# nexus-rl/dfd-starter

Measured on AMD Instinct MI355X. Metric: env steps/sec (whole node) + sec/FD-grad-step, 4096 antithetic perturbations, higher is better.
Workload: dtype f32; 1 GPU; BASELINE config 3: HalfCheetah-shaped synthetic env (obs 17, act 6), MujocoPolicy(17,6) P=6092, 4096 antithetic perturbations per GPU (2048 directions x +/-), T=1000 fixed-length episodes, full FD step (rollout + weights + gradient + DSGD); perturbations_per_gpu=4096, envs_per_perturbation=1, global_perturbations=4096, episode_len=1000, n_params=6092, parallelism=dp1

## Files before the change

### dfd-starter_amd/csrc/fdr_dpp_gen.h

```cpp
#pragma once

namespace fdr {

__device__ __forceinline__ void dpp_dot_32x1(float& a0, float X0, float X1, const float* w) {
  asm volatile(
      "s_nop 1\n\t"
      "v_mul_f32_dpp %0, %1, %3 row_newbcast:0 row_mask:0xf bank_mask:0xf\n\t"
      "v_fmac_f32_dpp %0, %2, %19 row_newbcast:0 row_mask:0xf bank_mask:0xf\n\t"
      "v_fmac_f32_dpp %0, %1, %4 row_newbcast:1 row_mask:0xf bank_mask:0xf\n\t"
      "v_fmac_f32_dpp %0, %2, %20 row_newbcast:1 row_mask:0xf bank_mask:0xf\n\t"
      "v_fmac_f32_dpp %0, %1, %5 row_newbcast:2 row_mask:0xf bank_mask:0xf\n\t"
      "v_fmac_f32_dpp %0, %2, %21 row_newbcast:2 row_mask:0xf bank_mask:0xf\n\t"
      "v_fmac_f32_dpp %0, %1, %6 row_newbcast:3 row_mask:0xf bank_mask:0xf\n\t"
      "v_fmac_f32_dpp %0, %2, %22 row_newbcast:3 row_mask:0xf bank_mask:0xf\n\t"
      "v_fmac_f32_dpp %0, %1, %7 row_newbcast:4 row_mask:0xf bank_mask:0xf\n\t"
      "v_fmac_f32_dpp %0, %2, %23 row_newbcast:4 row_mask:0xf bank_mask:0xf\n\t"
      "v_fmac_f32_dpp %0, %1, %8 row_newbcast:5 row_mask:0xf bank_mask:0xf\n\t"
      "v_fmac_f32_dpp %0, %2, %24 row_newbcast:5 row_mask:0xf bank_mask:0xf\n\t"
      "v_fmac_f32_dpp %0, %1, %9 row_newbcast:6 row_mask:0xf bank_mask:0xf\n\t"
      "v_fmac_f32_dpp %0, %2, %25 row_newbcast:6 row_mask:0xf bank_mask:0xf\n\t"
      "v_fmac_f32_dpp %0, %1, %10 row_newbcast:7 row_mask:0xf bank_mask:0xf\n\t"
      "v_fmac_f32_dpp %0, %2, %26 row_newbcast:7 row_mask:0xf bank_mask:0xf\n\t"
      "v_fmac_f32_dpp %0, %1, %11 row_newbcast:8 row_mask:0xf bank_mask:0xf\n\t"
      "v_fmac_f32_dpp %0, %2, %27 row_newbcast:8 row_mask:0xf bank_mask:0xf\n\t"
// ... 166 lines not shown
      "v_fmac_f32_dpp %0, %1, %11 row_newbcast:9 row_mask:0xf bank_mask:0xf\n\t"
      "v_fmac_f32_dpp %0, %1, %12 row_newbcast:10 row_mask:0xf bank_mask:0xf\n\t"
      : "+v"(a0)
      : "v"(X0), "v"(w[0]), "v"(w[1]), "v"(w[2]), "v"(w[3]), "v"(w[4]), "v"(w[5]), "v"(w[6]), "v"(w[7]), "v"(w[8]), "v"(w[9]), "v"(w[10]));
}
__device__ __forceinline__ void dpp_fma_tail12(float& a0, float X0, const float* w) {
  asm volatile(
      "s_nop 1\n\t"
      "v_fmac_f32_dpp %0, %1, %2 row_newbcast:0 row_mask:0xf bank_mask:0xf\n\t"
      "v_fmac_f32_dpp %0, %1, %3 row_newbcast:1 row_mask:0xf bank_mask:0xf\n\t"
      "v_fmac_f32_dpp %0, %1, %4 row_newbcast:2 row_mask:0xf bank_mask:0xf\n\t"
      "v_fmac_f32_dpp %0, %1, %5 row_newbcast:3 row_mask:0xf bank_mask:0xf\n\t"
      "v_fmac_f32_dpp %0, %1, %6 row_newbcast:4 row_mask:0xf bank_mask:0xf\n\t"
      "v_fmac_f32_dpp %0, %1, %7 row_newbcast:5 row_mask:0xf bank_mask:0xf\n\t"
      "v_fmac_f32_dpp %0, %1, %8 row_newbcast:6 row_mask:0xf bank_mask:0xf\n\t"
      "v_fmac_f32_dpp %0, %1, %9 row_newbcast:7 row_mask:0xf bank_mask:0xf\n\t"
      "v_fmac_f32_dpp %0, %1, %10 row_newbcast:8 row_mask:0xf bank_mask:0xf\n\t"
      "v_fmac_f32_dpp %0, %1, %11 row_newbcast:9 row_mask:0xf bank_mask:0xf\n\t"
      "v_fmac_f32_dpp %0, %1, %12 row_newbcast:10 row_mask:0xf bank_mask:0xf\n\t"
      "v_fmac_f32_dpp %0, %1, %13 row_newbcast:11 row_mask:0xf bank_mask:0xf\n\t"
      : "+v"(a0)
      : "v"(X0), "v"(w[0]), "v"(w[1]), "v"(w[2]), "v"(w[3]), "v"(w[4]), "v"(w[5]), "v"(w[6]), "v"(w[7]), "v"(w[8]), "v"(w[9]), "v"(w[10]), "v"(w[11]));
}
__device__ __forceinline__ void dpp_fma_tail13(float& a0, float X0, const float* w) {
  asm volatile(
      "s_nop 1\n\t"
      "v_fmac_f32_dpp %0, %1, %2 row_newbcast:0 row_mask:0xf bank_mask:0xf\n\t"
      "v_fmac_f32_dpp %0, %1, %3 row_newbcast:1 row_mask:0xf bank_mask:0xf\n\t"
      "v_fmac_f32_dpp %0, %1, %4 row_newbcast:2 row_mask:0xf bank_mask:0xf\n\t"
      "v_fmac_f32_dpp %0, %1, %5 row_newbcast:3 row_mask:0xf bank_mask:0xf\n\t"
      "v_fmac_f32_dpp %0, %1, %6 row_newbcast:4 row_mask:0xf bank_mask:0xf\n\t"
      "v_fmac_f32_dpp %0, %1, %7 row_newbcast:5 row_mask:0xf bank_mask:0xf\n\t"
      "v_fmac_f32_dpp %0, %1, %8 row_newbcast:6 row_mask:0xf bank_mask:0xf\n\t"
      "v_fmac_f32_dpp %0, %1, %9 row_newbcast:7 row_mask:0xf bank_mask:0xf\n\t"
      "v_fmac_f32_dpp %0, %1, %10 row_newbcast:8 row_mask:0xf bank_mask:0xf\n\t"
      "v_fmac_f32_dpp %0, %1, %11 row_newbcast:9 row_mask:0xf bank_mask:0xf\n\t"
      "v_fmac_f32_dpp %0, %1, %12 row_newbcast:10 row_mask:0xf bank_mask:0xf\n\t"
      "v_fmac_f32_dpp %0, %1, %13 row_newbcast:11 row_mask:0xf bank_mask:0xf\n\t"
      "v_fmac_f32_dpp %0, %1, %14 row_newbcast:12 row_mask:0xf bank_mask:0xf\n\t"
      : "+v"(a0)
      : "v"(X0), "v"(w[0]), "v"(w[1]), "v"(w[2]), "v"(w[3]), "v"(w[4]), "v"(w[5]), "v"(w[6]), "v"(w[7]), "v"(w[8]), "v"(w[9]), "v"(w[10]), "v"(w[11]), "v"(w[12]));
}
__device__ __forceinline__ void dpp_fma_tail14(float& a0, float X0, const float* w) {
  asm volatile(
      "s_nop 1\n\t"
      "v_fmac_f32_dpp %0, %1, %2 row_newbcast:0 row_mask:0xf bank_mask:0xf\n\t"
      "v_fmac_f32_dpp %0, %1, %3 row_newbcast:1 row_mask:0xf bank_mask:0xf\n\t"
      "v_fmac_f32_dpp %0, %1, %4 row_newbcast:2 row_mask:0xf bank_mask:0xf\n\t"
      "v_fmac_f32_dpp %0, %1, %5 row_newbcast:3 row_mask:0xf bank_mask:0xf\n\t"
      "v_fmac_f32_dpp %0, %1, %6 row_newbcast:4 row_mask:0xf bank_mask:0xf\n\t"
      "v_fmac_f32_dpp %0, %1, %7 row_newbcast:5 row_mask:0xf bank_mask:0xf\n\t"
      "v_fmac_f32_dpp %0, %1, %8 row_newbcast:6 row_mask:0xf bank_mask:0xf\n\t"
      "v_fmac_f32_dpp %0, %1, %9 row_newbcast:7 row_mask:0xf bank_mask:0xf\n\t"
      "v_fmac_f32_dpp %0, %1, %10 row_newbcast:8 row_mask:0xf bank_mask:0xf\n\t"
      "v_fmac_f32_dpp %0, %1, %11 row_newbcast:9 row_mask:0xf bank_mask:0xf\n\t"
      "v_fmac_f32_dpp %0, %1, %12 row_newbcast:10 row_mask:0xf bank_mask:0xf\n\t"
      "v_fmac_f32_dpp %0, %1, %13 row_newbcast:11 row_mask:0xf bank_mask:0xf\n\t"
      "v_fmac_f32_dpp %0, %1, %14 row_newbcast:12 row_mask:0xf bank_mask:0xf\n\t"
      "v_fmac_f32_dpp %0, %1, %15 row_newbcast:13 row_mask:0xf bank_mask:0xf\n\t"
      : "+v"(a0)
      : "v"(X0), "v"(w[0]), "v"(w[1]), "v"(w[2]), "v"(w[3]), "v"(w[4]), "v"(w[5]), "v"(w[6]), "v"(w[7]), "v"(w[8]), "v"(w[9]), "v"(w[10]), "v"(w[11]), "v"(w[12]), "v"(w[13]));
}
__device__ __forceinline__ void dpp_fma_tail15(float& a0, float X0, const float* w) {
  asm volatile(
      "s_nop 1\n\t"
      "v_fmac_f32_dpp %0, %1, %2 row_newbcast:0 row_mask:0xf bank_mask:0xf\n\t"
      "v_fmac_f32_dpp %0, %1, %3 row_newbcast:1 row_mask:0xf bank_mask:0xf\n\t"
      "v_fmac_f32_dpp %0, %1, %4 row_newbcast:2 row_mask:0xf bank_mask:0xf\n\t"
      "v_fmac_f32_dpp %0, %1, %5 row_newbcast:3 row_mask:0xf bank_mask:0xf\n\t"
      "v_fmac_f32_dpp %0, %1, %6 row_newbcast:4 row_mask:0xf bank_mask:0xf\n\t"
      "v_fmac_f32_dpp %0, %1, %7 row_newbcast:5 row_mask:0xf bank_mask:0xf\n\t"
      "v_fmac_f32_dpp %0, %1, %8 row_newbcast:6 row_mask:0xf bank_mask:0xf\n\t"
      "v_fmac_f32_dpp %0, %1, %9 row_newbcast:7 row_mask:0xf bank_mask:0xf\n\t"
      "v_fmac_f32_dpp %0, %1, %10 row_newbcast:8 row_mask:0xf bank_mask:0xf\n\t"
      "v_fmac_f32_dpp %0, %1, %11 row_newbcast:9 row_mask:0xf bank_mask:0xf\n\t"
      "v_fmac_f32_dpp %0, %1, %12 row_newbcast:10 row_mask:0xf bank_mask:0xf\n\t"
      "v_fmac_f32_dpp %0, %1, %13 row_newbcast:11 row_mask:0xf bank_mask:0xf\n\t"
      "v_fmac_f32_dpp %0, %1, %14 row_newbcast:12 row_mask:0xf bank_mask:0xf\n\t"
      "v_fmac_f32_dpp %0, %1, %15 row_newbcast:13 row_mask:0xf bank_mask:0xf\n\t"
      "v_fmac_f32_dpp %0, %1, %16 row_newbcast:14 row_mask:0xf bank_mask:0xf\n\t"
      : "+v"(a0)
      : "v"(X0), "v"(w[0]), "v"(w[1]), "v"(w[2]), "v"(w[3]), "v"(w[4]), "v"(w[5]), "v"(w[6]), "v"(w[7]), "v"(w[8]), "v"(w[9]), "v"(w[10]), "v"(w[11]), "v"(w[12]), "v"(w[13]), "v"(w[14]));
}
}
```

### dfd-starter_amd/csrc/fdr_mlp_pair.h

```cpp
#pragma once
#include "fdr_mlp.h"

namespace fdr {

constexpr int kPairWaves = 2;

__device__ __forceinline__ f2 tanh2_pre(f2 t) {
  const f2 d = f2{__builtin_amdgcn_exp2f(t.x), __builtin_amdgcn_exp2f(t.y)} + f2{1.f, 1.f};
  return pk_fma(f2{-2.f, -2.f}, f2{__builtin_amdgcn_rcpf(d.x), __builtin_amdgcn_rcpf(d.y)}, f2{1.f, 1.f});
}
__device__ __forceinline__ f2 tanh2_fast(f2 x) {
  return tanh2_pre(x * f2{kTanhScale, kTanhScale});
}
constexpr float kPreScale = kTanhScale;
template <bool kPre>
__device__ __forceinline__ f2 tanh2_act(f2 z) {
  if constexpr (kPre) return tanh2_pre(z);
  else return tanh2_fast(z);
}

template <int NIN, int NA, bool DISC>
struct MlpPair {
  using L = Layout<NIN, NA, DISC>;
  static constexpr int NOUT = L::NOUT;
  static constexpr int NX = round4(NIN);
  static_assert(NX <= 32, "pair kernel: policy input wider than 32");
  static constexpr bool kBiasCol = NIN < NX;
  static constexpr bool kW1Lds = NIN > 8;
  static constexpr bool kPre = !DISC;
  static constexpr float kWS = kPre ? kTanhScale : 1.f;
  static constexpr int kW1Chunks = kW1Lds ? NX / 4 : 0;
  static constexpr int kTileF4 = (2 * kW1Chunks + 8) * kWave;
  f2 w1a[kW1Lds ? 1 : NX / 2], w1b[kW1Lds ? 1 : NX / 2];
  float b1a, b1b;
  const float4* tile;
  f2 w2[64];
  float b2a, b2b, b3;
  float a0, c0, a1a, c1a, a1b, c1b, a2a, c2a, a2b, c2b;

  __host__ __device__ static constexpr int head_unit(int rho, int k, int e) {
    return 32 * rho + 8 * (k >> 2) + 4 * e + (k & 3);
  }

  template <class Src>
  __device__ __forceinline__ void load(Src& src, int t, int tid, const float* bn_mean, const float* bn_var,
                                       float4* wave_tile) {
    const int rho = t >> 4, o = t & 15;
    const int ua = 2 * t, ub = 2 * t + 1;
    float4* my = wave_tile + tid;
    tile = my;
    auto w1v = [&](int u, int k) {
      return kWS * (k < NIN ? src.get(L::L1W + (int64_t)u * NIN + k) : (k == NIN ? src.get(L::L1B + u) : 0.f));
    };
    if constexpr (kPk) {
#pragma unroll
      for (int j = 0; j < 2 * kW1Chunks; ++j) {
        const float e0 = w1v(ua, 2 * j), f0 = w1v(ub, 2 * j), e1 = w1v(ua, 2 * j + 1), f1 = w1v(ub, 2 * j + 1);
        my[j * kWave] = float4{e0, f0, e1, f1};
      }
    } else if constexpr (kW1Lds) {
#pragma unroll
      for (int m = 0; m < kW1Chunks; ++m) {
        const float e0 = w1v(ua, 4 * m), e1 = w1v(ua, 4 * m + 1), e2 = w1v(ua, 4 * m + 2), e3 = w1v(ua, 4 * m + 3);
        my[m * kWave] = float4{e0, e1, e2, e3};
        const float f0 = w1v(ub, 4 * m), f1 = w1v(ub, 4 * m + 1), f2_ = w1v(ub, 4 * m + 2), f3 = w1v(ub, 4 * m + 3);
        my[(kW1Chunks + m) * kWave] = float4{f0, f1, f2_, f3};
      }
    } else {
#pragma unroll
      for (int p = 0; p < NX / 2; ++p) {
        const float e0 = w1v(ua, 2 * p), e1 = w1v(ua, 2 * p + 1);
        w1a[p] = f2{e0, e1};
        const float f0 = w1v(ub, 2 * p), f1 = w1v(ub, 2 * p + 1);
        w1b[p] = f2{f0, f1};
      }
    }
    b1a = kBiasCol ? 0.f : kWS * src.get(L::L1B + ua);
    b1b = kBiasCol ? 0.f : kWS * src.get(L::L1B + ub);
    __builtin_amdgcn_sched_barrier(0);
    const int q4 = t >> 2, c4 = t & 3;
#pragma unroll
    for (int p = 0; p < 4; ++p) {
      const int row0 = 8 * q4 + (c4 ^ p), row1 = row0 + 4;
#pragma unroll
      for (int k = 0; k < 16; ++k) {
        const float e0 = src.get(L::L2W + (int64_t)row0 * kHidden + 16 * c4 + k);
        const float e1 = src.get(L::L2W + (int64_t)row1 * kHidden + 16 * c4 + k);
        w2[p * 16 + k] = f2{kWS * e0, kWS * e1};
      }
#pragma unroll
      for (int k = 0; k < 16; ++k) asm volatile("" : "+v"(w2[p * 16 + k]));
      asm volatile("" : "+v"(src.n2));
      __builtin_amdgcn_sched_barrier(0);
    }
    const int u2a = 8 * q4 + c4, u2b = 8 * q4 + 4 + c4;
    b2a = kWS * src.get(L::L2B + u2a);
    b2b = kWS * src.get(L::L2B + u2b);
    {
      const bool has_o = o < NOUT;
      const int oc = has_o ? o : 0;
#pragma unroll
      for (int m = 0; m < 8; ++m) {
        float e[4];
#pragma unroll
        for (int i = 0; i < 4; ++i) {
          const int w = 4 * m + i;
          e[i] = src.get_if(L::L3W + (int64_t)oc * kHidden + head_unit(rho, w & 15, w >> 4), has_o);
        }
        my[(2 * kW1Chunks + m) * kWave] =
            has_o ? float4{kWS * e[0], kWS * e[1], kWS * e[2], kWS * e[3]} : float4{0.f, 0.f, 0.f, 0.f};
      }
      const float b3v = src.get_if(L::L3B + oc, has_o && rho == 0);
      b3 = has_o ? kWS * b3v : 0.f;
    }
    wave_lds_sync();
    a0 = c0 = a1a = c1a = a1b = c1b = a2a = c2a = a2b = c2b = 0.f;
    if constexpr (DISC) {
      const float* bm = bn_mean ? bn_mean : src.base;
      const float* bv = bn_var ? bn_var : src.base;
      auto stat = [&](int k, float& rm, float& rv) {
        const float m = bm[k], v = bv[k];
        rm = bn_mean ? m : 0.f;
        rv = bn_var ? v : 1.f;
      };
      {
        const bool in = t < NIN;
        const int tc = in ? t : 0;
        const float w = src.get_if(L::BN0W + tc, in), b = src.get_if(L::BN0B + tc, in);
        float rm, rv, a, c;
        stat(tc, rm, rv);
        bn_fold(w, b, rm, rv, a, c);
        a0 = in ? a : 0.f;
        c0 = in ? c : 0.f;
      }
      auto fold = [&](int64_t wofs, int64_t bofs, int st, int u, float& av, float& cv) {
        const float w = src.get(wofs + u), b = src.get(bofs + u);
        float rm, rv;
        stat(st + u, rm, rv);
        bn_fold(w, b, rm, rv, av, cv);
      };
      fold(L::BN1W, L::BN1B, NIN, ua, a1a, c1a);
      fold(L::BN1W, L::BN1B, NIN, ub, a1b, c1b);
      fold(L::BN2W, L::BN2B, NIN + kHidden, u2a, a2a, c2a);
      fold(L::BN2W, L::BN2B, NIN + kHidden, u2b, a2b, c2b);
    }
  }

  __device__ __forceinline__ float input_transform(float x) const {
    if constexpr (DISC) {
      return fmaf(x, a0, c0);
    } else {
      return x;
    }
  }

  __device__ __forceinline__ float act1(float z, float av, float cv) const {
    if constexpr (DISC) {
      return fmaf(fmaxf(z, 0.f), av, cv);
    } else {
      return tanh_act<kPre>(z);
    }
  }

  static constexpr bool kTail = kW1Lds && kBiasCol && NX - NIN == 3;
  static constexpr int NQ = kTail ? NX / 4 - 1 : NX / 4;
  static constexpr bool kPk = kW1Lds && kBiasCol;
  static constexpr int kPkPairs = (NIN + 2) / 2;
  struct L1Rows {
    float4 wa[kW1Lds && !kPk ? NQ : 1], wb[kW1Lds && !kPk ? NQ : 1], m[NQ];
    float2 ta, tb;
    float tm;
    float4 wp[kPk ? kPkPairs : 1];
  };
  __device__ __forceinline__ void l1_prefetch(L1Rows& r, const float* mrow) const {
    const float4* m4 = reinterpret_cast<const float4*>(mrow);
#pragma unroll
    for (int q = 0; q < NQ; ++q) {
      if constexpr (kW1Lds && !kPk) {
        r.wa[q] = tile[q * kWave];
        r.wb[q] = tile[(kW1Chunks + q) * kWave];
      }
// ... 43 lines not shown
    const f2 am = am0 + am1;
    return am.x + am.y;
  }
  __device__ __forceinline__ f2 layer1_q(const SIn& xin, const L1Rows& rows) const {
    const float xt = xin.t;
    auto xq = [&](int q) { return xin.v[q]; };
    f2 aa0 = {b1a, 0.f}, aa1 = {0.f, 0.f}, ab0 = {b1b, 0.f}, ab1 = {0.f, 0.f};
    if constexpr (kPk) {
      constexpr int NC = 2;
      f2 acc[NC];
#pragma unroll
      for (int q = 0; q < NC; ++q) acc[q] = f2{0.f, 0.f};
#pragma unroll
      for (int q = 0; q < NQ; ++q) {
        const float4 xv = xq(q);
#pragma unroll
        for (int i = 0; i < 4; ++i) {
          const int k = 4 * q + i;
          if (k < NIN) {
            const float4 w = rows.wp[k >> 1];
            const f2 xp = (i < 2) ? f2{xv.x, xv.y} : f2{xv.z, xv.w};
            if (kPre && k == NIN % NC) {
              const float4 wb = rows.wp[NIN >> 1];
              const f2 bias = (NIN & 1) ? f2{wb.z, wb.w} : f2{wb.x, wb.y};
              acc[k % NC] = (k & 1) ? pk_fma_bhi(f2{w.z, w.w}, xp, bias) : pk_fma_blo(f2{w.x, w.y}, xp, bias);
            } else if (k < NC)
              acc[k % NC] = (k & 1) ? pk_mul_bhi(f2{w.z, w.w}, xp) : pk_mul_blo(f2{w.x, w.y}, xp);
            else
              acc[k % NC] = (k & 1) ? pk_fma_bhi(f2{w.z, w.w}, xp, acc[k % NC]) : pk_fma_blo(f2{w.x, w.y}, xp, acc[k % NC]);
          }
        }
      }
      if constexpr (kTail) {
        const float4 w = rows.wp[(NIN - 1) >> 1];
        acc[(NIN - 1) % NC] = pk_fma(((NIN - 1) & 1) ? f2{w.z, w.w} : f2{w.x, w.y}, f2{xt, xt}, acc[(NIN - 1) % NC]);
      }
      if constexpr (!kPre || NIN % NC >= NIN) {
        const float4 w = rows.wp[NIN >> 1];
        acc[NIN % NC] = acc[NIN % NC] + ((NIN & 1) ? f2{w.z, w.w} : f2{w.x, w.y});
      }
      const f2 h = acc[0] + acc[1];
      if constexpr (DISC) {
        return f2{act1(h.x, a1a, c1a), act1(h.y, a1b, c1b)};
      } else {
        return tanh2_act<kPre>(h);
      }
    }
#pragma unroll
    for (int q = 0; q < NQ; ++q) {
      const float4 xv = xq(q);
      float4 wa, wb;
      if constexpr (kW1Lds) {
        wa = rows.wa[q];
        wb = rows.wb[q];
      } else {
        wa = float4{w1a[2 * q].x, w1a[2 * q].y, w1a[2 * q + 1].x, w1a[2 * q + 1].y};
        wb = float4{w1b[2 * q].x, w1b[2 * q].y, w1b[2 * q + 1].x, w1b[2 * q + 1].y};
      }
      aa0 = pk_fma(f2{wa.x, wa.y}, f2{xv.x, xv.y}, aa0);
      ab0 = pk_fma(f2{wb.x, wb.y}, f2{xv.x, xv.y}, ab0);
      aa1 = pk_fma(f2{wa.z, wa.w}, f2{xv.z, xv.w}, aa1);
      ab1 = pk_fma(f2{wb.z, wb.w}, f2{xv.z, xv.w}, ab1);
    }
    if constexpr (kTail) {
      aa1 = pk_fma(f2{rows.ta.x, rows.ta.y}, f2{xt, 1.f}, aa1);
      ab1 = pk_fma(f2{rows.tb.x, rows.tb.y}, f2{xt, 1.f}, ab1);
    }
    const f2 ha = aa0 + aa1, hb = ab0 + ab1;
    if constexpr (DISC) {
      return f2{act1(ha.x + ha.y, a1a, c1a), act1(hb.x + hb.y, a1b, c1b)};
    } else {
      return tanh2_act<kPre>(f2{ha.x + ha.y, hb.x + hb.y});
    }
  }

  template <class Mark>
  __device__ __forceinline__ float layers23(f2 h1, float* h1s, int t, Mark&& mark) const {
    const int c4 = t & 3;
    float x[16];
    reinterpret_cast<f2*>(h1s)[t] = h1;
    __builtin_amdgcn_s_setprio(0);
    wave_lds_sync();
    lds_bcast<16>(h1s + 16 * c4, x);
    float w3[32];
#pragma unroll
    for (int m = 0; m < 8; ++m) {
      const float4 w = tile[(2 * kW1Chunks + m) * kWave];
      w3[4 * m] = w.x;
      w3[4 * m + 1] = w.y;
      w3[4 * m + 2] = w.z;
      w3[4 * m + 3] = w.w;
    }
    f2 acc[4];
#pragma unroll
    for (int p = 0; p < 4; ++p)
      acc[p] = pk_fma(w2[p * 16], f2{x[0], x[0]}, (kPre && p == 0) ? f2{b2a, b2b} : f2{0.f, 0.f});
    {
      f2 xp[8];
#pragma unroll
      for (int j = 0; j < 8; ++j) xp[j] = f2{x[2 * j], x[2 * j + 1]};
#define FDR_L2_HI "op_sel:[0,1,0] op_sel_hi:[1,1,1]"
#define FDR_L2_LO "op_sel_hi:[1,0,1]"
      asm(
          "v_pk_fma_f32 %0, %4, %64, %0 " FDR_L2_HI "\n"
          "v_pk_fma_f32 %1, %5, %64, %1 " FDR_L2_HI "\n"
          "v_pk_fma_f32 %2, %6, %64, %2 " FDR_L2_HI "\n"
          "v_pk_fma_f32 %3, %7, %64, %3 " FDR_L2_HI "\n"
          "v_pk_fma_f32 %0, %8, %65, %0 " FDR_L2_LO "\n"
          "v_pk_fma_f32 %1, %9, %65, %1 " FDR_L2_LO "\n"
          "v_pk_fma_f32 %2, %10, %65, %2 " FDR_L2_LO "\n"
          "v_pk_fma_f32 %3, %11, %65, %3 " FDR_L2_LO "\n"
          "v_pk_fma_f32 %0, %12, %65, %0 " FDR_L2_HI "\n"
          "v_pk_fma_f32 %1, %13, %65, %1 " FDR_L2_HI "\n"
          "v_pk_fma_f32 %2, %14, %65, %2 " FDR_L2_HI "\n"
          "v_pk_fma_f32 %3, %15, %65, %3 " FDR_L2_HI "\n"
          "v_pk_fma_f32 %0, %16, %66, %0 " FDR_L2_LO "\n"
          "v_pk_fma_f32 %1, %17, %66, %1 " FDR_L2_LO "\n"
          "v_pk_fma_f32 %2, %18, %66, %2 " FDR_L2_LO "\n"
          "v_pk_fma_f32 %3, %19, %66, %3 " FDR_L2_LO "\n"
          "v_pk_fma_f32 %0, %20, %66, %0 " FDR_L2_HI "\n"
          "v_pk_fma_f32 %1, %21, %66, %1 " FDR_L2_HI "\n"
          "v_pk_fma_f32 %2, %22, %66, %2 " FDR_L2_HI "\n"
          "v_pk_fma_f32 %3, %23, %66, %3 " FDR_L2_HI "\n"
          "v_pk_fma_f32 %0, %24, %67, %0 " FDR_L2_LO "\n"
          "v_pk_fma_f32 %1, %25, %67, %1 " FDR_L2_LO "\n"
          "v_pk_fma_f32 %2, %26, %67, %2 " FDR_L2_LO "\n"
          "v_pk_fma_f32 %3, %27, %67, %3 " FDR_L2_LO "\n"
          "v_pk_fma_f32 %0, %28, %67, %0 " FDR_L2_HI "\n"
          "v_pk_fma_f32 %1, %29, %67, %1 " FDR_L2_HI "\n"
          "v_pk_fma_f32 %2, %30, %67, %2 " FDR_L2_HI "\n"
          "v_pk_fma_f32 %3, %31, %67, %3 " FDR_L2_HI "\n"
          "v_pk_fma_f32 %0, %32, %68, %0 " FDR_L2_LO "\n"
          "v_pk_fma_f32 %1, %33, %68, %1 " FDR_L2_LO "\n"
          "v_pk_fma_f32 %2, %34, %68, %2 " FDR_L2_LO "\n"
          "v_pk_fma_f32 %3, %35, %68, %3 " FDR_L2_LO "\n"
          "v_pk_fma_f32 %0, %36, %68, %0 " FDR_L2_HI "\n"
          "v_pk_fma_f32 %1, %37, %68, %1 " FDR_L2_HI "\n"
          "v_pk_fma_f32 %2, %38, %68, %2 " FDR_L2_HI "\n"
          "v_pk_fma_f32 %3, %39, %68, %3 " FDR_L2_HI "\n"
          "v_pk_fma_f32 %0, %40, %69, %0 " FDR_L2_LO "\n"
          "v_pk_fma_f32 %1, %41, %69, %1 " FDR_L2_LO "\n"
          "v_pk_fma_f32 %2, %42, %69, %2 " FDR_L2_LO "\n"
          "v_pk_fma_f32 %3, %43, %69, %3 " FDR_L2_LO "\n"
          "v_pk_fma_f32 %0, %44, %69, %0 " FDR_L2_HI "\n"
          "v_pk_fma_f32 %1, %45, %69, %1 " FDR_L2_HI "\n"
          "v_pk_fma_f32 %2, %46, %69, %2 " FDR_L2_HI "\n"
          "v_pk_fma_f32 %3, %47, %69, %3 " FDR_L2_HI "\n"
          "v_pk_fma_f32 %0, %48, %70, %0 " FDR_L2_LO "\n"
          "v_pk_fma_f32 %1, %49, %70, %1 " FDR_L2_LO "\n"
          "v_pk_fma_f32 %2, %50, %70, %2 " FDR_L2_LO "\n"
          "v_pk_fma_f32 %3, %51, %70, %3 " FDR_L2_LO "\n"
          "v_pk_fma_f32 %0, %52, %70, %0 " FDR_L2_HI "\n"
          "v_pk_fma_f32 %1, %53, %70, %1 " FDR_L2_HI "\n"
          "v_pk_fma_f32 %2, %54, %70, %2 " FDR_L2_HI "\n"
          "v_pk_fma_f32 %3, %55, %70, %3 " FDR_L2_HI "\n"
          "v_pk_fma_f32 %0, %56, %71, %0 " FDR_L2_LO "\n"
          "v_pk_fma_f32 %1, %57, %71, %1 " FDR_L2_LO "\n"
          "v_pk_fma_f32 %2, %58, %71, %2 " FDR_L2_LO "\n"
          "v_pk_fma_f32 %3, %59, %71, %3 " FDR_L2_LO "\n"
          "v_pk_fma_f32 %3, %63, %71, %3 " FDR_L2_HI "\n"
          "v_pk_fma_f32 %2, %62, %71, %2 " FDR_L2_HI "\n"
          "v_pk_fma_f32 %0, %60, %71, %0 " FDR_L2_HI "\n"
          "v_pk_fma_f32 %1, %61, %71, %1 " FDR_L2_HI "\n"
          : "+v"(acc[0]), "+v"(acc[1]), "+v"(acc[2]), "+v"(acc[3])
          : "v"(w2[1]), "v"(w2[17]), "v"(w2[33]), "v"(w2[49]),
            "v"(w2[2]), "v"(w2[18]), "v"(w2[34]), "v"(w2[50]),
            "v"(w2[3]), "v"(w2[19]), "v"(w2[35]), "v"(w2[51]),
            "v"(w2[4]), "v"(w2[20]), "v"(w2[36]), "v"(w2[52]),
            "v"(w2[5]), "v"(w2[21]), "v"(w2[37]), "v"(w2[53]),
            "v"(w2[6]), "v"(w2[22]), "v"(w2[38]), "v"(w2[54]),
            "v"(w2[7]), "v"(w2[23]), "v"(w2[39]), "v"(w2[55]),
            "v"(w2[8]), "v"(w2[24]), "v"(w2[40]), "v"(w2[56]),
            "v"(w2[9]), "v"(w2[25]), "v"(w2[41]), "v"(w2[57]),
            "v"(w2[10]), "v"(w2[26]), "v"(w2[42]), "v"(w2[58]),
            "v"(w2[11]), "v"(w2[27]), "v"(w2[43]), "v"(w2[59]),
            "v"(w2[12]), "v"(w2[28]), "v"(w2[44]), "v"(w2[60]),
            "v"(w2[13]), "v"(w2[29]), "v"(w2[45]), "v"(w2[61]),
            "v"(w2[14]), "v"(w2[30]), "v"(w2[46]), "v"(w2[62]),
            "v"(w2[15]), "v"(w2[31]), "v"(w2[47]), "v"(w2[63]),
            "v"(xp[0]), "v"(xp[1]), "v"(xp[2]), "v"(xp[3]), "v"(xp[4]), "v"(xp[5]), "v"(xp[6]), "v"(xp[7]));
#undef FDR_L2_LO
#undef FDR_L2_HI
    }
    f2 zs;
    __builtin_amdgcn_s_setprio(1);
    {
      float o0, o1, o2, o3;
      asm volatile(
          "v_add_f32_dpp %2, %10, %6 quad_perm:[2,3,0,1] row_mask:0xf bank_mask:0xf bound_ctrl:1\n\t"
          "v_add_f32_dpp %3, %11, %7 quad_perm:[2,3,0,1] row_mask:0xf bank_mask:0xf bound_ctrl:1\n\t"
          "v_add_f32_dpp %0, %8, %4 quad_perm:[2,3,0,1] row_mask:0xf bank_mask:0xf bound_ctrl:1\n\t"
          "v_add_f32_dpp %1, %9, %5 quad_perm:[2,3,0,1] row_mask:0xf bank_mask:0xf bound_ctrl:1\n\t"
          "v_add_f32_dpp %0, %2, %0 quad_perm:[1,0,3,2] row_mask:0xf bank_mask:0xf bound_ctrl:1\n\t"
          "v_add_f32_dpp %1, %3, %1 quad_perm:[1,0,3,2] row_mask:0xf bank_mask:0xf bound_ctrl:1\n\t"
          : "=&v"(o0), "=&v"(o1), "=&v"(o2), "=&v"(o3)
          : "v"(acc[0].x), "v"(acc[0].y), "v"(acc[1].x), "v"(acc[1].y), "v"(acc[2].x), "v"(acc[2].y), "v"(acc[3].x),
            "v"(acc[3].y));
      zs = f2{o0, o1};
    }
    const float za = kPre ? zs.x : zs.x + b2a;
    const float zb = kPre ? zs.y : zs.y + b2b;
    mark(1, za);
    float h2a, h2b;
    if constexpr (DISC) {
      h2a = fmaf(fmaxf(za, 0.f), a2a, c2a);
      h2b = fmaf(fmaxf(zb, 0.f), a2b, c2b);
    } else {
      const f2 h2 = tanh2_act<kPre>(f2{za, zb});
      h2a = h2.x;
      h2b = h2.y;
    }
    float u;
    dpp_dot_32x1(u, h2a, h2b, w3);
    float v = u;
    permlane16_swap(u, v);
    const float out = (u + v) + b3;
    mark(2, out);
    return out;
  }

  template <bool kAll = false, bool kFast = false>
  __device__ __forceinline__ float softmax(float logit, int t) const {
    const bool valid = (t & 15) < NOUT;
    const float v = valid ? logit : -FLT_MAX;
    const float mx = row16_max_n<NOUT>(v);
    if constexpr (kFast) {
      const float e = valid ? __builtin_amdgcn_exp2f((v - mx) * 1.44269504088896341f) : 0.f;
      return e * __builtin_amdgcn_rcpf(row16_sum_n<NOUT>(e));
    } else {
      const float e = valid ? expf(v - mx) : 0.f;
      return e / row16_sum_n<NOUT>(e);
    }
  }
};

struct alignas(16) PairScratch {
  float h1[2][kHidden];
  float x[2][32];
};

template <int K>
__device__ __forceinline__ float row_bcast(float v) {
  return __builtin_bit_cast(float, __builtin_amdgcn_mov_dpp(__builtin_bit_cast(int, v), 0x150 + K, 0xF, 0xF, false));
}

template <int N, int... I>
__device__ __forceinline__ void row_bcast_all(float v, float (&out)[N], std::integer_sequence<int, I...>) {
  ((out[I] = row_bcast<I>(v)), ...);
}

}
```

### dfd-starter_amd/csrc/fdr_rollout_pair.hip

```cpp
#include <algorithm>

#include "fdr_mlp_pair.h"

namespace fdr {

#ifndef FDR_STEP_LOOP_PAD
#define FDR_STEP_LOOP_PAD 15
#endif
#if FDR_STEP_LOOP_PAD >= 0
#define FDR_STR2(x) #x
#define FDR_STR(x) FDR_STR2(x)
#define FDR_STEP_LOOP_PLACED asm volatile(".p2align 6\n\t.rept " FDR_STR(FDR_STEP_LOOP_PAD) "\n\ts_nop 0\n\t.endr");
#else
#define FDR_STEP_LOOP_PLACED
#endif

template <int NIN, int NA, bool DISC, int FEAT>
__global__ __launch_bounds__(64 * kPairWaves, 2) void rollout_pair_kernel(RolloutArgs a) {
  using Lane = MlpPair<NIN, NA, DISC>;
  constexpr int NX = Lane::NX;
  constexpr int NMK = NX + round4(NA);
  constexpr int MKS = NMK % 8 == 0 ? NMK + 4 : NMK;
  __shared__ float4 env4[NIN * MKS / 4];
  __shared__ float4 wtile[kPairWaves * Lane::kTileF4];
  __shared__ PairScratch scratch[kPairWaves];
  float* envMK = reinterpret_cast<float*>(env4);
  for (int e = threadIdx.x; e < NIN * MKS; e += blockDim.x) {
    const int i = e / MKS, k = e % MKS;
    envMK[e] = kPreScale * (k < NIN ? a.M[i * NIN + k] : (k >= NX && k < NX + NA ? a.K[i * NA + k - NX] : 0.f));
  }
  __syncthreads();

  const int tid = threadIdx.x & 63, wv = threadIdx.x >> 6, hh = tid >> 5, t = tid & 31;
  const int lane0 = a.lane_base + (blockIdx.x * kPairWaves + wv) * 2;
  if (lane0 >= a.n_lanes) return;
  const bool active = lane0 + hh < a.n_lanes;
  const int lane = active ? lane0 + hh : lane0;

  ParamSrc src = a.lanes.src(lane);
  const bool det = a.lanes.deterministic ? a.lanes.deterministic[lane] != 0 : false;
  Lane pl;
  pl.load(src, t, tid, a.bn_mean, a.bn_var, wtile + wv * Lane::kTileF4);
  {
    double n2 = src.n2;
#pragma unroll
    for (int m = 16; m >= 1; m >>= 1) n2 += __shfl_xor(n2, m, kWave);
    asm volatile("" : "+v"(n2));
    if (t == 0 && active && a.norm2) a.norm2[lane] = n2;
  }

  const int ji = t < NIN ? t : NIN - 1;
  constexpr bool norm_obs = (FEAT & kFeatObsNorm) != 0;
  const float om = norm_obs ? a.obs_mean[ji] : 0.f;
  const float osd = norm_obs ? a.obs_std[ji] : 1.f;
  auto policy_input = [&](float s) {
    float x = s;
    if (norm_obs) x = fminf(fmaxf((s - om) / osd, -10.f), 10.f);
    return pl.input_transform(x);
  };
  float s = a.s0[ji];
  const int T = a.T;
  const uint64_t key = a.key;
  const uint64_t ulane = (uint64_t)(a.lanes.lane_offset + lane);
  double racc = 0.0;
  float eacc = 0.f;
  const int o = t & 15;
  constexpr int kDrawsPerStep = DISC ? 1 : NA;
  constexpr int kStepsPerBatch = 32 / kDrawsPerStep;
  constexpr bool kTerm = (FEAT & kFeatTerm) != 0;
  bool alive0 = true, alive1 = true;
  int n0 = T, n1 = T;
  auto alive_me = [&]() { return hh ? alive1 : alive0; };
  float rbuf = 0.f;
  const int zbase = 4 * (32 * hh + (DISC ? 0 : (o < NA ? o : 0)));
  auto* sc = &scratch[wv];
  [[maybe_unused]] float* xs = sc->x[hh];
  float* h1s = sc->h1[hh];
  const float* mrow = envMK + ji * MKS;
  constexpr bool kSame = !DISC && !norm_obs;
  typename Lane::L1Rows l1rows;
  pl.l1_prefetch(l1rows, mrow);
  float kr[DISC ? 1 : NA];
#pragma unroll
  for (int m = 0; m < (DISC ? 1 : NA); ++m) kr[m] = mrow[NX + m];
  int tb = 0;
#ifdef FDR_PHASE_STAMPS
  uint64_t ph_acc[5] = {0, 0, 0, 0, 0};
  uint64_t ph_last = 0;
  auto mark = [&](int k, float dep) {
    uint64_t now;
    asm volatile("s_memtime %0\n\ts_waitcnt lgkmcnt(0)" : "=s"(now) : "v"(dep));
    if (k >= 0) ph_acc[k] += now - ph_last;
    ph_last = now;
  };
#else
  auto mark = [](int, float) {};
#endif
  auto draw = [&](int st) {
    const int ds = t / kDrawsPerStep, dk = t % kDrawsPerStep;
    const uint64_t hsh = hash_ctr(key, ulane, (uint64_t)(st + ds), (uint64_t)dk);
    rbuf = DISC ? uniform24(hsh) : normal_bm(hsh);
  };
  int dctr = ((t / kDrawsPerStep) << 4) | (t % kDrawsPerStep);
  uint64_t dz = 0;
  float du1 = 0.f, du2 = 0.f;
  auto draw_part = [&](int k, int st) {
    if (k == 0) {
      asm volatile("" : "+v"(dctr)::"memory");
      dz = mix64_a(key + (((uint64_t)ulane << 32) | (uint64_t)((st << 4) + dctr)) * 0x9E3779B97F4A7C15ull);
    } else if (k == 1) {
      asm volatile("" : "+v"(dz)::"memory");
      dz = mix64_b(dz);
    } else if (k == 2) {
      asm volatile("" : "+v"(dz)::"memory");
      const uint64_t hsh = mix64_c(dz);
      du1 = bm_u1(hsh);
      du2 = bm_u2(hsh);
    } else if (k == 3) {
      asm volatile("" : "+v"(du1)::"memory");
      du1 = bm_radius(du1);
    } else if (k == 4) {
      asm volatile("" : "+v"(du1), "+v"(du2)::"memory");
      rbuf = bm_normal(du1, du2);
    }
  };
  auto step = [&](int st, int tb, auto&& fill) {
    const float zt = __builtin_bit_cast(
        float, __builtin_amdgcn_ds_bpermute(zbase + 4 * kDrawsPerStep * tb, __builtin_bit_cast(int, rbuf)));
    if constexpr (FEAT & kFeatStates) {
      if (t < NIN && active && (!kTerm || alive_me())) a.states[((int64_t)lane * T + st) * NIN + t] = s;
    }
    float pre = 0.f;
    xs[t] = t < NIN ? policy_input(s) : (t == NIN ? 1.f : 0.f);
    if constexpr (!kSame) h1s[t] = t < NIN ? s : 0.f;
    wave_lds_sync();
    typename Lane::SIn sin;
    const f2 h1 = pl.template layer1_env<kSame>(xs, h1s, l1rows, sin, fill);
    pre = pl.env_ms(sin, l1rows);

    mark(0, h1.x);
    const float y = pl.layers23(h1, h1s, t, mark);
    pl.l1_prefetch(l1rows, mrow);
    if constexpr (DISC) {
      const float p = det ? pl.softmax(y, t) : pl.template softmax<false, true>(y, t);
      float pv[NA];
      row_bcast_all(p, pv, std::make_integer_sequence<int, NA>{});
      float tot = 0.f;
#pragma unroll
      for (int i = 0; i < NA; ++i) tot += pv[i];
      int act_d = 0;
      if (det) {
        float best = pv[0];
#pragma unroll
        for (int i = 1; i < NA; ++i) {
          act_d = pv[i] > best ? i : act_d;
          best = fmaxf(best, pv[i]);
        }
      } else {
        const float target = zt * tot;
        float cs = 0.f;
#pragma unroll
        for (int i = 0; i < NA - 1; ++i) {
          cs += pv[i];
          act_d += cs <= target ? 1 : 0;
        }
      }
      eacc -= (o < NA && (!kTerm || alive_me())) ? disc_entropy_term(p, tot) : 0.f;
      pre += mrow[NX + act_d];
    } else {
      const float th = tanh_act<Lane::kPre>(y);
      const float sd = std_from_tanh(dpp_mov<kDppRowShl + NA>(th));
      if constexpr (kTerm)
        eacc += alive_me() ? __builtin_amdgcn_logf(sd) : 0.f;
      else
        eacc += __builtin_amdgcn_logf(sd);
      const float act_c = det ? th : gauss_action(th, sd, zt);
      mark(3, act_c);
      dpp_tail<NA>(pre, act_c, kr);
    }
    s = tanh_pre(pre);
    mark(4, s);
    if constexpr (kTerm) {
      racc += alive_me() ? (double)s : 0.0;
      const bool d0 = fabsf(readlane_f(s, a.done_dim)) > a.done_thr;
      const bool d1 = fabsf(readlane_f(s, 32 + a.done_dim)) > a.done_thr;
      if (alive0 && d0) {
        alive0 = false;
        n0 = st + 1;
      }
      if (alive1 && d1) {
        alive1 = false;
        n1 = st + 1;
      }
      return !alive0 && !alive1;
    } else {
      racc += (double)s;
      return false;
    }
  };
  if constexpr (!DISC) {
    [&] {
      int st = 0;
      draw(0);
      FDR_STEP_LOOP_PLACED
      for (; st + kStepsPerBatch <= T; st += kStepsPerBatch) {
        asm volatile("" ::: "memory");
        mark(-1, s);
#pragma unroll
        for (int k = 0; k < kStepsPerBatch; ++k) {
          if (k) {
            asm volatile("" ::: "memory");
            mark(-1, s);
          }
          constexpr int kLast = kStepsPerBatch - 1;
          static_assert(kLast >= 4, "draw_part: five parts need a batch of five steps");
          const int part = k == kLast ? 4 : (k < 4 ? k : -1);
          if (step(st + k, k, [&] { draw_part(part, st + kStepsPerBatch); })) return;
        }
      }
      if (st < T) {
        for (int k = 0; st + k < T; ++k) {
          asm volatile("" ::: "memory");
          mark(-1, s);
          if (step(st + k, k, [] {})) return;
        }
      }
    }();
  } else {
    for (int st = 0; st < T; ++st) {
      asm volatile("" ::: "memory");
      mark(-1, s);
      if (!det && tb == 0) draw(st);
      if (step(st, tb, [] {})) break;
      tb = tb + 1 == kStepsPerBatch ? 0 : tb + 1;
    }
  }

#ifdef FDR_PHASE_STAMPS
  if (blockIdx.x == 0 && threadIdx.x == 0)
    for (int k = 0; k < 5; ++k) g_phase_stamps[k] = ph_acc[k];
#endif
  eacc *= 0.693147180559945309f;
  double esum = (t < NA) ? (double)eacc : 0.0;
#pragma unroll
  for (int m = 16; m >= 1; m >>= 1) esum += __shfl_xor(esum, m, kWave);
  if (t == 0 && active) {
    double r = racc;
    if (a.jiggle) r += (hash_ctr(key, ulane, kJiggleT, 15) & 1ull) ? 1e-12 : -1e-12;
    a.ret[lane] = r;
    const int nsteps = hh ? n1 : n0;
    double e = esum / (double)nsteps;
    if constexpr (!DISC) e += (double)NA * 1.4189385332046727;
    a.ent[lane] = e;
    a.steps[lane] = nsteps;
  }
}

int launch_rollout_pair(const PolicyKey& k, const RolloutArgs& args, int round_lanes, hipStream_t stream) {
  return with_shape<false>(k, "no compiled rollout for this (kind, n_in, n_act)", [&](auto shape) {
    using S = decltype(shape);
    FDR_PHASE_UNIT();
    const int quantum = 2 * kPairWaves;
    const int n_rounds = round_lanes > 0 ? (args.n_lanes + round_lanes - 1) / round_lanes : 1;
    const int per = ((args.n_lanes + n_rounds - 1) / n_rounds + quantum - 1) / quantum * quantum;
    const int feat = rollout_feat(args, args.done_thr > 0.f);
    RolloutArgs r = args;
    for (int base = 0; base < args.n_lanes; base += per) {
      r.lane_base = base;
      const dim3 grid((std::min(per, args.n_lanes - base) + quantum - 1) / quantum), block(64 * kPairWaves);
      const bool hit = launch_feat_set<kPairFeatBits>(feat, [&](auto f) {
        hipLaunchKernelGGL((rollout_pair_kernel<S::NIN, S::NA, S::DISC, decltype(f)::value>), grid, block, 0, stream,
                           r);
      });
      if (!hit) return set_error(FDR_ERR_UNSUPPORTED, "no compiled rollout_pair_kernel for this feature set");
    }
    return check_launch("rollout_pair_kernel<synth>");
  });
}

}
```

### dfd-starter_amd/csrc/fdr_wave.h

```cpp
#pragma once
#include <hip/hip_runtime.h>

#include "fdr_dpp_gen.h"

namespace fdr {

__device__ __forceinline__ void permlane32_swap(float& a, float& b) {
  asm volatile("s_nop 1\n\tv_permlane32_swap_b32 %0, %1" : "+v"(a), "+v"(b));
}
__device__ __forceinline__ void permlane16_swap(float& a, float& b) {
  asm volatile("s_nop 1\n\tv_permlane16_swap_b32 %0, %1" : "+v"(a), "+v"(b));
}

__device__ __forceinline__ float row_allreduce_sum(float v) {
  float a = v, b = v;
  permlane32_swap(a, b);
  float s = a + b;
  float c = s, d = s;
  permlane16_swap(c, d);
  return c + d;
}

template <int N>
__device__ __forceinline__ void dpp_tail(float& acc, float X, const float* w) {
  static_assert(N >= 0 && N < 16, "tail of 0..15 inputs");
  if constexpr (N == 1) dpp_fma_tail1(acc, X, w);
  if constexpr (N == 2) dpp_fma_tail2(acc, X, w);
  if constexpr (N == 3) dpp_fma_tail3(acc, X, w);
  if constexpr (N == 4) dpp_fma_tail4(acc, X, w);
  if constexpr (N == 5) dpp_fma_tail5(acc, X, w);
  if constexpr (N == 6) dpp_fma_tail6(acc, X, w);
  if constexpr (N == 7) dpp_fma_tail7(acc, X, w);
  if constexpr (N == 8) dpp_fma_tail8(acc, X, w);
  if constexpr (N == 9) dpp_fma_tail9(acc, X, w);
  if constexpr (N == 10) dpp_fma_tail10(acc, X, w);
  if constexpr (N == 11) dpp_fma_tail11(acc, X, w);
  if constexpr (N == 12) dpp_fma_tail12(acc, X, w);
  if constexpr (N == 13) dpp_fma_tail13(acc, X, w);
  if constexpr (N == 14) dpp_fma_tail14(acc, X, w);
  if constexpr (N == 15) dpp_fma_tail15(acc, X, w);
}

__device__ __forceinline__ float dot_row16(float v, const float* w) {
  float a0, a1, a2, a3;
  dpp_dot_16x4(a0, a1, a2, a3, v, w);
  return (a0 + a2) + (a1 + a3);
}

template <int CTRL>
__device__ __forceinline__ float dpp_mov(float v) {
  return __builtin_bit_cast(float, __builtin_amdgcn_mov_dpp(__builtin_bit_cast(int, v), CTRL, 0xF, 0xF, true));
}
constexpr int kDppQuadXor1 = 0xB1;
constexpr int kDppQuadXor2 = 0x4E;
constexpr int kDppHalfMirror = 0x141;
constexpr int kDppMirror = 0x140;
constexpr int kDppRowShl = 0x100;
constexpr int kDppRowRor = 0x120;

__device__ __forceinline__ float row16_max(float v) {
  v = fmaxf(v, dpp_mov<kDppQuadXor1>(v));
  v = fmaxf(v, dpp_mov<kDppQuadXor2>(v));
  v = fmaxf(v, dpp_mov<kDppHalfMirror>(v));
  v = fmaxf(v, dpp_mov<kDppMirror>(v));
  return v;
}
__device__ __forceinline__ float row16_sum(float v) {
  v += dpp_mov<kDppQuadXor1>(v);
  v += dpp_mov<kDppQuadXor2>(v);
  v += dpp_mov<kDppHalfMirror>(v);
  v += dpp_mov<kDppMirror>(v);
  return v;
}

template <int N>
__device__ __forceinline__ float row16_max_n(float v) {
  if constexpr (N == 2) {
    float m;
    asm volatile("s_nop 1\n\tv_max_f32_dpp %0, %1, %1 quad_perm:[1,0,3,2] row_mask:0xf bank_mask:0xf bound_ctrl:1"
                 : "=v"(m) : "v"(v));
    return m;
  }
  v = fmaxf(v, dpp_mov<kDppQuadXor1>(v));
  if constexpr (N > 2) v = fmaxf(v, dpp_mov<kDppQuadXor2>(v));
  if constexpr (N > 4) v = fmaxf(v, dpp_mov<kDppHalfMirror>(v));
  if constexpr (N > 8) v = fmaxf(v, dpp_mov<kDppMirror>(v));
  return v;
}
template <int N>
__device__ __forceinline__ float row16_sum_n(float v) {
  v += dpp_mov<kDppQuadXor1>(v);
  if constexpr (N > 2) v += dpp_mov<kDppQuadXor2>(v);
  if constexpr (N > 4) v += dpp_mov<kDppHalfMirror>(v);
  if constexpr (N > 8) v += dpp_mov<kDppMirror>(v);
  return v;
}

__device__ __forceinline__ float readlane_f(float v, int lane) {
  return __builtin_bit_cast(float, __builtin_amdgcn_readlane(__builtin_bit_cast(int, v), lane));
}

}
```

Before: 4.674 billion env steps/s.

## Use reduce-scatter head layout for 12-output continuous policy layer 3

For continuous policies with 12 outputs (6 means plus 6 stds), the layer-3 head changes from a 32-FMA broadcast DPP dot product to a reduce-scatter scheme. It uses 12 packed multiply/FMAs followed by a DPP butterfly reduction, with a permuted weight-slot layout checked by a static_assert. This cuts the per-lane weight tile from 8 to 6 float4 chunks and shrinks the layer-3 instruction count. In exchange, the action outputs move to lanes 0,1,2,4,5,6, so the std shift, action tail DPP and entropy lane selection all have to change. The new asm also hardcodes VGPRs v232-v243, which can constrain register allocation.

```diff
diff --git a/dfd-starter_amd/csrc/fdr_dpp_gen.h b/dfd-starter_amd/csrc/fdr_dpp_gen.h
--- a/dfd-starter_amd/csrc/fdr_dpp_gen.h
+++ b/dfd-starter_amd/csrc/fdr_dpp_gen.h
@@ -272,4 +272,82 @@
       : "+v"(a0)
       : "v"(X0), "v"(w[0]), "v"(w[1]), "v"(w[2]), "v"(w[3]), "v"(w[4]), "v"(w[5]), "v"(w[6]), "v"(w[7]), "v"(w[8]), "v"(w[9]), "v"(w[10]), "v"(w[11]), "v"(w[12]), "v"(w[13]), "v"(w[14]));
 }
-}
+__device__ __forceinline__ void dpp_fma_tail6_q3(float& a0, float X0, const float* w) {
+  asm volatile(
+      "s_nop 1\n\t"
+      "v_fmac_f32_dpp %0, %1, %2 row_newbcast:0 row_mask:0xf bank_mask:0xf\n\t"
+      "v_fmac_f32_dpp %0, %1, %3 row_newbcast:1 row_mask:0xf bank_mask:0xf\n\t"
+      "v_fmac_f32_dpp %0, %1, %4 row_newbcast:2 row_mask:0xf bank_mask:0xf\n\t"
+      "v_fmac_f32_dpp %0, %1, %5 row_newbcast:4 row_mask:0xf bank_mask:0xf\n\t"
+      "v_fmac_f32_dpp %0, %1, %6 row_newbcast:5 row_mask:0xf bank_mask:0xf\n\t"
+      "v_fmac_f32_dpp %0, %1, %7 row_newbcast:6 row_mask:0xf bank_mask:0xf\n\t"
+      : "+v"(a0)
+      : "v"(X0), "v"(w[0]), "v"(w[1]), "v"(w[2]), "v"(w[3]), "v"(w[4]), "v"(w[5]));
+}
+typedef float dpp_f2 __attribute__((ext_vector_type(2)));
+constexpr unsigned char kHeadRs12Slot[16][12] = {
+    {0, 1, 2, 5, 3, 4, 11, 9, 10, 6, 7, 8},
+    {1, 0, 2, 5, 4, 3, 11, 10, 9, 7, 6, 8},
+    {2, 1, 0, 4, 3, 5, 10, 9, 11, 8, 7, 6},
+    {2, 0, 1, 3, 4, 5, 9, 10, 11, 8, 6, 7},
+    {3, 4, 5, 2, 0, 1, 8, 6, 7, 9, 10, 11},
+    {4, 3, 5, 2, 1, 0, 8, 7, 6, 10, 9, 11},
+    {5, 4, 3, 1, 0, 2, 7, 6, 8, 11, 10, 9},
+    {5, 3, 4, 0, 1, 2, 6, 7, 8, 11, 9, 10},
+    {6, 7, 8, 11, 9, 10, 5, 3, 4, 0, 1, 2},
+    {7, 6, 8, 11, 10, 9, 5, 4, 3, 1, 0, 2},
+    {8, 7, 6, 10, 9, 11, 4, 3, 5, 2, 1, 0},
+    {8, 6, 7, 9, 10, 11, 3, 4, 5, 2, 0, 1},
+    {9, 10, 11, 8, 6, 7, 2, 0, 1, 3, 4, 5},
+    {10, 9, 11, 8, 7, 6, 2, 1, 0, 4, 3, 5},
+    {11, 10, 9, 7, 6, 8, 1, 0, 2, 5, 4, 3},
+    {11, 9, 10, 6, 7, 8, 0, 1, 2, 5, 3, 4},
+};
+__host__ __device__ constexpr int head_rs12_out(int l) { return 3 * (l >> 2) + ((l & 3) < 2 ? (l & 3) : 2); }
+__host__ __device__ constexpr int head_rs12_slot(int l, int r) {
+  const int lp = l ^ (r < 3 ? 0 : (r < 6 ? 7 : (r < 9 ? 15 : 8)));
+  return 3 * (lp >> 2) + ((0x486864 >> (2 * (3 * (lp & 3) + r % 3))) & 3);
+}
+constexpr bool head_rs12_table_ok() {
+  for (int l = 0; l < 16; ++l)
+    for (int r = 0; r < 12; ++r)
+      if (kHeadRs12Slot[l][r] != head_rs12_slot(l, r)) return false;
+  return true;
+}
+static_assert(head_rs12_table_ok(), "head_rs12_slot != kHeadRs12Slot");
+__device__ __forceinline__ void dpp_head_rs12(float& u, float& v, const dpp_f2* w, dpp_f2 h) {
+  asm volatile(
+      "v_pk_mul_f32 v[232:233], %2, %14 op_sel_hi:[1,0]\n\t"
+      "v_pk_mul_f32 v[234:235], %3, %14 op_sel_hi:[1,0]\n\t"
+      "v_pk_mul_f32 v[236:237], %4, %14 op_sel_hi:[1,0]\n\t"
+      "v_pk_mul_f32 v[238:239], %5, %14 op_sel_hi:[1,0]\n\t"
+      "v_pk_mul_f32 v[240:241], %6, %14 op_sel_hi:[1,0]\n\t"
+      "v_pk_mul_f32 v[242:243], %7, %14 op_sel_hi:[1,0]\n\t"
+      "v_pk_fma_f32 v[238:239], %11, %14, v[238:239] op_sel:[0,1,0] op_sel_hi:[1,1,1]\n\t"
+      "v_pk_fma_f32 v[240:241], %12, %14, v[240:241] op_sel:[0,1,0] op_sel_hi:[1,1,1]\n\t"
+      "v_pk_fma_f32 v[242:243], %13, %14, v[242:243] op_sel:[0,1,0] op_sel_hi:[1,1,1]\n\t"
+      "v_pk_fma_f32 v[232:233], %8, %14, v[232:233] op_sel:[0,1,0] op_sel_hi:[1,1,1]\n\t"
+      "v_pk_fma_f32 v[234:235], %9, %14, v[234:235] op_sel:[0,1,0] op_sel_hi:[1,1,1]\n\t"
+      "v_pk_fma_f32 v[236:237], %10, %14, v[236:237] op_sel:[0,1,0] op_sel_hi:[1,1,1]\n\t"
+      "v_add_f32_dpp v235, v241, v235 row_mirror row_mask:0xf bank_mask:0xf bound_ctrl:1\n\t"
+      "v_add_f32_dpp v236, v242, v236 row_mirror row_mask:0xf bank_mask:0xf bound_ctrl:1\n\t"
+      "v_add_f32_dpp v237, v243, v237 row_mirror row_mask:0xf bank_mask:0xf bound_ctrl:1\n\t"
+      "v_add_f32_dpp v232, v238, v232 row_mirror row_mask:0xf bank_mask:0xf bound_ctrl:1\n\t"
+      "v_add_f32_dpp v233, v239, v233 row_mirror row_mask:0xf bank_mask:0xf bound_ctrl:1\n\t"
+      "v_add_f32_dpp v234, v240, v234 row_mirror row_mask:0xf bank_mask:0xf bound_ctrl:1\n\t"
+      "v_add_f32_dpp v234, v237, v234 row_half_mirror row_mask:0xf bank_mask:0xf bound_ctrl:1\n\t"
+      "v_add_f32_dpp v233, v236, v233 row_half_mirror row_mask:0xf bank_mask:0xf bound_ctrl:1\n\t"
+      "v_add_f32_dpp v232, v235, v232 row_half_mirror row_mask:0xf bank_mask:0xf bound_ctrl:1\n\t"
+      "v_add_f32_dpp v232, v234, v232 quad_perm:[2,3,0,1] row_mask:0xf bank_mask:0xf bound_ctrl:1\n\t"
+      "v_add_f32_dpp v233, v233, v233 quad_perm:[2,3,0,1] row_mask:0xf bank_mask:0xf bound_ctrl:1\n\t"
+      "v_cndmask_b32_e64 v234, v233, v232, %15\n\t"
+      "s_nop 1\n\t"
+      "v_add_f32_dpp v233, v234, v232 quad_perm:[1,0,3,2] row_mask:0xf bank_mask:0xf bound_ctrl:1\n\t"
+      "v_add_f32_dpp v232, v234, v232 quad_perm:[1,0,3,2] row_mask:0xf bank_mask:0xf bound_ctrl:1\n\t"
+      "s_nop 1\n\t"
+      "v_permlane16_swap_b32 v232, v233\n\t"
+      : "=&{v232}"(u), "=&{v233}"(v)
+      : "v"(w[0]), "v"(w[1]), "v"(w[2]), "v"(w[3]), "v"(w[4]), "v"(w[5]), "v"(w[6]), "v"(w[7]), "v"(w[8]), "v"(w[9]), "v"(w[10]), "v"(w[11]), "v"(h), "s"(0xccccccccccccccccull)
+      : "v234", "v235", "v236", "v237", "v238", "v239", "v240", "v241", "v242", "v243");
+}
+}
diff --git a/dfd-starter_amd/csrc/fdr_mlp_pair.h b/dfd-starter_amd/csrc/fdr_mlp_pair.h
--- a/dfd-starter_amd/csrc/fdr_mlp_pair.h
+++ b/dfd-starter_amd/csrc/fdr_mlp_pair.h
@@ -30,7 +30,9 @@
   static constexpr bool kPre = !DISC;
   static constexpr float kWS = kPre ? kTanhScale : 1.f;
   static constexpr int kW1Chunks = kW1Lds ? NX / 4 : 0;
-  static constexpr int kTileF4 = (2 * kW1Chunks + 8) * kWave;
+  static constexpr bool kHeadRS = !DISC && NOUT == 12;
+  static constexpr int kW3Chunks = kHeadRS ? 6 : 8;
+  static constexpr int kTileF4 = (2 * kW1Chunks + kW3Chunks) * kWave;
   f2 w1a[kW1Lds ? 1 : NX / 2], w1b[kW1Lds ? 1 : NX / 2];
   float b1a, b1b;
   const float4* tile;
@@ -96,7 +98,17 @@
     const int u2a = 8 * q4 + c4, u2b = 8 * q4 + 4 + c4;
     b2a = kWS * src.get(L::L2B + u2a);
     b2b = kWS * src.get(L::L2B + u2b);
-    {
+    if constexpr (kHeadRS) {
+#pragma unroll
+      for (int m = 0; m < 6; ++m) {
+        float e[4];
+#pragma unroll
+        for (int i = 0; i < 4; ++i)
+          e[i] = src.get(L::L3W + (int64_t)head_rs12_slot(o, 4 * (m % 3) + i) * kHidden + (m < 3 ? u2a : u2b));
+        my[(2 * kW1Chunks + m) * kWave] = float4{kWS * e[0], kWS * e[1], kWS * e[2], kWS * e[3]};
+      }
+      b3 = kWS * src.get_if(L::L3B + head_rs12_out(o), rho == 0 && c4 != 3);
+    } else {
       const bool has_o = o < NOUT;
       const int oc = has_o ? o : 0;
 #pragma unroll
@@ -306,9 +318,9 @@
     __builtin_amdgcn_s_setprio(0);
     wave_lds_sync();
     lds_bcast<16>(h1s + 16 * c4, x);
-    float w3[32];
-#pragma unroll
-    for (int m = 0; m < 8; ++m) {
+    float w3[4 * kW3Chunks];
+#pragma unroll
+    for (int m = 0; m < kW3Chunks; ++m) {
       const float4 w = tile[(2 * kW1Chunks + m) * kWave];
       w3[4 * m] = w.x;
       w3[4 * m + 1] = w.y;
@@ -434,10 +446,17 @@
       h2a = h2.x;
       h2b = h2.y;
     }
-    float u;
-    dpp_dot_32x1(u, h2a, h2b, w3);
-    float v = u;
-    permlane16_swap(u, v);
+    float u, v;
+    if constexpr (kHeadRS) {
+      f2 w3p[12];
+#pragma unroll
+      for (int j = 0; j < 12; ++j) w3p[j] = f2{w3[2 * j], w3[2 * j + 1]};
+      dpp_head_rs12(u, v, w3p, f2{h2a, h2b});
+    } else {
+      dpp_dot_32x1(u, h2a, h2b, w3);
+      v = u;
+      permlane16_swap(u, v);
+    }
     const float out = (u + v) + b3;
     mark(2, out);
     return out;
diff --git a/dfd-starter_amd/csrc/fdr_rollout_pair.hip b/dfd-starter_amd/csrc/fdr_rollout_pair.hip
--- a/dfd-starter_amd/csrc/fdr_rollout_pair.hip
+++ b/dfd-starter_amd/csrc/fdr_rollout_pair.hip
@@ -72,7 +72,11 @@
   int n0 = T, n1 = T;
   auto alive_me = [&]() { return hh ? alive1 : alive0; };
   float rbuf = 0.f;
-  const int zbase = 4 * (32 * hh + (DISC ? 0 : (o < NA ? o : 0)));
+  constexpr bool kRS = Lane::kHeadRS;
+  constexpr int kStdShl = kRS ? 8 : NA;
+  int zbase;
+  if constexpr (kRS) zbase = 4 * (32 * hh + ((o < 8 && (o & 3) != 3) ? o - (o >> 2) : 0));
+  else zbase = 4 * (32 * hh + (DISC ? 0 : (o < NA ? o : 0)));
   auto* sc = &scratch[wv];
   [[maybe_unused]] float* xs = sc->x[hh];
   float* h1s = sc->h1[hh];
@@ -169,14 +173,15 @@
       pre += mrow[NX + act_d];
     } else {
       const float th = tanh_act<Lane::kPre>(y);
-      const float sd = std_from_tanh(dpp_mov<kDppRowShl + NA>(th));
+      const float sd = std_from_tanh(dpp_mov<kDppRowShl + kStdShl>(th));
       if constexpr (kTerm)
         eacc += alive_me() ? __builtin_amdgcn_logf(sd) : 0.f;
       else
         eacc += __builtin_amdgcn_logf(sd);
       const float act_c = det ? th : gauss_action(th, sd, zt);
       mark(3, act_c);
-      dpp_tail<NA>(pre, act_c, kr);
+      if constexpr (kRS) dpp_tail_q3<NA>(pre, act_c, kr);
+      else dpp_tail<NA>(pre, act_c, kr);
     }
     s = tanh_pre(pre);
     mark(4, s);
@@ -241,7 +246,9 @@
     for (int k = 0; k < 5; ++k) g_phase_stamps[k] = ph_acc[k];
 #endif
   eacc *= 0.693147180559945309f;
-  double esum = (t < NA) ? (double)eacc : 0.0;
+  double esum;
+  if constexpr (kRS) esum = (t < 8 && (t & 3) != 3) ? (double)eacc : 0.0;
+  else esum = (t < NA) ? (double)eacc : 0.0;
 #pragma unroll
   for (int m = 16; m >= 1; m >>= 1) esum += __shfl_xor(esum, m, kWave);
   if (t == 0 && active) {
diff --git a/dfd-starter_amd/csrc/fdr_wave.h b/dfd-starter_amd/csrc/fdr_wave.h
--- a/dfd-starter_amd/csrc/fdr_wave.h
+++ b/dfd-starter_amd/csrc/fdr_wave.h
@@ -39,6 +39,12 @@
   if constexpr (N == 13) dpp_fma_tail13(acc, X, w);
   if constexpr (N == 14) dpp_fma_tail14(acc, X, w);
   if constexpr (N == 15) dpp_fma_tail15(acc, X, w);
+}
+
+template <int N>
+__device__ __forceinline__ void dpp_tail_q3(float& acc, float X, const float* w) {
+  static_assert(N == 6, "generated for 6 inputs (lanes 0, 1, 2, 4, 5, 6)");
+  dpp_fma_tail6_q3(acc, X, w);
 }
 
 __device__ __forceinline__ float dot_row16(float v, const float* w) {
```

Result: faster. 4.732 billion env steps/s, median of 6 (+1.2%).
